# ns1labs/pktvisor

Hardware: AMD Instinct MI355X
Metric: Mpkt/s device-resident (Net+DNS handler parse) (higher is better)
Workload: dtype u8; 1 GPU; C2: Net+DNS handlers, 64 B UDP (Eth+IPv4+UDP+22 B), Zipf IPs, host_spec 10.x.x.x/8; records_per_gpu=10000000, handlers=net v1 + dns v1 (default groups), parallelism=dp1

## Files before the change

pktvisor_amd/csrc/pv_host.cpp:

```cpp
#include "pv_host.h"

namespace {

int parse_host_spec(pv_ctx *c, const char *spec)
{
    if (!spec) return 0;
    std::string s = spec;
    size_t pos = 0;
    while (pos < s.size()) {
        size_t e = s.find(',', pos);
        std::string host = s.substr(pos, e == std::string::npos ? std::string::npos : e - pos);
        pos = e == std::string::npos ? s.size() : e + 1;
        if (host.empty()) continue;
        size_t d = host.find('/');
        if (d == std::string::npos) return c->fail(PV_EINVAL, "invalid CIDR: %s", host.c_str());
        std::string ip = host.substr(0, d), cs = host.substr(d + 1);
        if (cs.empty() || !std::all_of(cs.begin(), cs.end(), ::isdigit)) return c->fail(PV_EINVAL, "invalid CIDR: %s", host.c_str());
        int cidr = atoi(cs.c_str());
        if (ip.find(':') != std::string::npos) {
            if (cidr < 0 || cidr > 128) return c->fail(PV_EINVAL, "invalid CIDR: %s", host.c_str());
            if (c->nets.n6 >= PV_MAX_SUBNETS) return c->fail(PV_EINVAL, "too many host subnets");
            uint8_t a[16];
            if (inet_pton(AF_INET6, ip.c_str(), a) != 1) return c->fail(PV_EINVAL, "invalid IPv6 address: %s", ip.c_str());
            memcpy(c->nets.v6_addr[c->nets.n6], a, 16);
// ... 2568 lines not shown
    if (status[ST_FLAGS] & PVF_NAMES_PENDING) {
        for (uint32_t t = 0; t < PV_TABLES; t++)
            hipLaunchKernelGGL(pv_topn_name_fix, dim3((uint32_t)c->cus * 4), dim3(256), 0, st, (const PvParams *)c->d_params, t);
        if (!hip_ok(e = hipGetLastError()) || !hip_ok(e = hipStreamSynchronize(st))) return c->hipfail(e, "pending names");
        if (getenv("PV_NAMEFIX_TRACE")) fprintf(stderr, "pv: pending top-N names written (pv_topn_name_fix)\n");
    }
    HP(4);
    {
        float ms = 0;
        if (timed && hipEventElapsedTime(&ms, c->ev_start, c->ev_stop) == hipSuccess) { c->kernel_ms += ms; c->kernel_launches++; }
    }
    if (!c->tcp_pre) {
        if (int rc = tcp_stage(c, d_recs, d_offs, n, status[ST_TSEG], status[ST_TSEG_BYTES], first_sec, false, st)) return rc;
    }
    const uint32_t gt = tcp_pass(c, P, a, a + nord, st, c->h_params + 1);
    if (gt) {
        if (P.want_events)
            hipLaunchKernelGGL(pv_xact_compact, dim3(gt), dim3(256), 0, st, (const PvParams *)c->d_params, grid,
                               status[ST_NKEYS]);
        if (!hip_ok(e = hipGetLastError())) return c->hipfail(e, "launch pv_dns_tcp");
        if (!hip_ok(e = hipMemcpyAsync(c->h_status, c->d_status, ST_RB_WORDS * 4, hipMemcpyDeviceToHost, st)) ||
            !hip_ok(e = hipStreamSynchronize(st)))
            return c->hipfail(e, "TCP DNS pass");
        memcpy(status, c->h_status, sizeof status);
    }
    for (uint32_t k = 0; k <= P.n_shift; k++) c->net.clean[P.slot_of[k]] = false;
    if (status[ST_NDNS] || gt)
        for (uint32_t k = 0; k <= P.n_dshift; k++) c->dns.clean[P.dslot_of[k]] = false;
    bool drained = false;
    if (int rc = drain_overflow(c, st, true, &drained)) return rc;
    uint32_t flags = status[ST_FLAGS];
    if (drained && !hip_ok(e = hipMemcpy(&flags, c->d_status + ST_FLAGS, 4, hipMemcpyDeviceToHost))) return c->hipfail(e, "status");
    if (flags & PVF_TABLE_FULL) return c->fail(PV_ECAPACITY, "top-N table full: raise table_log2");
    if (flags & PVF_ARENA_FULL) return c->fail(PV_ECAPACITY, "top-N name arena full");
    if (getenv("PV_TSTAMPS")) {
        std::vector<uint64_t> tv(65536 + (2u << c->reg_log2) * 8);
        if (hip_ok(hipMemcpy(tv.data(), c->d_stamps + (1u << 20), tv.size() * 8, hipMemcpyDeviceToHost))) {
            double cs[8] = {0}, ms[8] = {0};
            uint64_t nm = 0;
            const uint32_t cg = P.cb_grid;
            for (uint32_t w = 0; w < cg; w++)
                for (int k = 0; k < 8; k++) cs[k] += (double)tv[w * 8 + k];
            for (uint32_t w = 0; w < (2u << c->reg_log2); w++) {
                const uint64_t *m = &tv[65536 + w * 8];
                if (!m[0] && !m[1]) continue;
                nm++;
                for (int k = 0; k < 8; k++) ms[k] += (double)m[k];
            }
            fprintf(stderr, "pv_tstamps combine (%u wg): init=%.0f insert=%.0f count=%.0f scan=%.0f out=%.0f | merge (%lu wg): "
                            "runs=%.0f load=%.0f insert=%.0f names=%.0f wb=%.0f\n",
                    cg, cs[0] / cg, cs[1] / cg, cs[2] / cg, cs[3] / cg, cs[4] / cg, (unsigned long)nm,
                    ms[0] / std::max<uint64_t>(nm, 1), ms[1] / std::max<uint64_t>(nm, 1), ms[2] / std::max<uint64_t>(nm, 1),
                    ms[3] / std::max<uint64_t>(nm, 1), ms[4] / std::max<uint64_t>(nm, 1));
            hipMemset(c->d_stamps + (1u << 20), 0, tv.size() * 8);
        }
        std::vector<uint64_t> nv((size_t)reg_grid * 4);
        int khz = 0;
        hipDeviceGetAttribute(&khz, hipDeviceAttributeWallClockRate, c->device);
        if (lean && hip_ok(hipMemcpy(nv.data(), c->d_stamps + (1u << 20) + (1u << 18), nv.size() * 8, hipMemcpyDeviceToHost)) && nv[0]) {
            uint64_t first = ~0ull;
            std::vector<uint32_t> xcc(reg_grid);
            for (uint32_t w = 0; w < reg_grid; w++) {
                xcc[w] = (uint32_t)(nv[w * 4] >> 60);
                nv[w * 4] &= ~(0xfull << 60);
                first = std::min(first, nv[w * 4]);
            }
            const double us = khz > 0 ? 1000.0 / khz : 0.01;
            fprintf(stderr, "pv_tstamps net (%u wg, %s):", reg_grid, fuse ? "fused" : "pair");
            static const char *nm[4] = {"start", "net_end", "handover", "end"};
            for (int k = 0; k < (fuse ? 4 : 2); k++) {
                std::vector<double> v;
                for (uint32_t w = 0; w < reg_grid; w++)
                    if (nv[w * 4 + k]) v.push_back((double)(nv[w * 4 + k] - first) * us);
                if (v.empty()) continue;
                std::sort(v.begin(), v.end());
                fprintf(stderr, " %s min=%.2f med=%.2f max=%.2f us", nm[k], v.front(), v[v.size() / 2], v.back());
            }
            fprintf(stderr, "\n");
            fprintf(stderr, "pv_tstamps net_end by xcc:");
            for (uint32_t x = 0; x < 16; x++) {
                std::vector<double> v;
                for (uint32_t w = 0; w < reg_grid; w++)
                    if (xcc[w] == x && nv[w * 4 + 1]) v.push_back((double)(nv[w * 4 + 1] - first) * us);
                if (v.empty()) continue;
                std::sort(v.begin(), v.end());
                fprintf(stderr, " x%u(n=%zu) %.0f/%.0f/%.0f", x, v.size(), v.front(), v[v.size() / 2], v.back());
            }
            fprintf(stderr, "\n");
            hipMemset(c->d_stamps + (1u << 20) + (1u << 18), 0, nv.size() * 8);
        }
    }
    if (getenv("PV_STAMPS")) {
        std::vector<uint64_t> stv((size_t)grid * 4 * 8);
        if (hip_ok(hipMemcpy(stv.data(), c->d_stamps, stv.size() * 8, hipMemcpyDeviceToHost))) {
            double sum[8] = {0};
            for (size_t w = 0; w < (size_t)grid * 4; w++)
                for (int k = 0; k < 8; k++) sum[k] += (double)stv[w * 8 + k];
            fprintf(stderr, "pv_stamps (mean cycles per wave, %u wave tiles/wg):", P.wt_per_block);
            static const char *nm[8] = {"slot", "commit", "barA", "issue", "parse", "lane", "barB", "flush"};
            for (int k = 0; k < 8; k++) fprintf(stderr, " %s=%.0f", nm[k], sum[k] / (grid * 4.0));
            fprintf(stderr, "\n");
        }
    }
    HP(5);
    if (int rc = pair_stage(c, P, status[ST_NEV], status[ST_NKEYS], status[ST_NRESP], n, st,
                            (uint64_t)(grid + gt) * P.wt_per_block * 64u))
        return rc;
// ... 1757 lines not shown
```

pktvisor_amd/csrc/pv_kernels.hip:

```cpp
#include <cstring>
#include <hip/hip_runtime.h>
#include <rocprim/rocprim.hpp>
#include <stdint.h>

#include "pv_layout.h"
#include "pv_geodb.h"

#define PV_BLOCK 256
#define PV_C __attribute__((address_space(4)))
#ifdef PV_STAMPS
#define STAMP_DECL                                                                           \
    uint64_t st_acc[8] = {0, 0, 0, 0, 0, 0, 0, 0};                                          \
    uint64_t st_prev = __builtin_amdgcn_s_memtime();
#define STAMP(k)                                                                             \
    {                                                                                        \
        const uint64_t now = __builtin_amdgcn_s_memtime();                                   \
        st_acc[k] += now - st_prev;                                                          \
        st_prev = now;                                                                       \
    }
#define STAMP_FLUSH                                                                          \
    if ((threadIdx.x & 63) == 0)                                                             \
        for (int k_ = 0; k_ < 8; k_++) P.stamps[((uint64_t)blockIdx.x * (blockDim.x / 64) + threadIdx.x / 64) * 8 + k_] = st_acc[k_];
#else
#define STAMP_DECL
// ... 1719 lines not shown
    Parsed o;
    o.caplen = f.caplen;
    o.sec = r.w[0];
    o.nsec = ts_nano ? (int32_t)r.w[1] : (int32_t)(r.w[1] * 1000u);
    o.frame = off + 16;
    o.l3 = 4; o.l4 = (uint8_t)f.l4; o.has4 = 1; o.has6 = 0; o.syn = (uint8_t)f.syn; o.dir = (uint8_t)f.dir;
    o.v4 = o.frame + 14; o.v6 = 0;
    o.l4off = f.l4 ? o.frame + 34 : 0;
    o.l4len = f.l4 ? f.l4len : 0;
    return o;
}
__device__ __forceinline__ SlowOut net_slow_p(const PvParams *__restrict__ Pp, const SAcc R, uint64_t off, uint64_t i)
{
    PV_CREF(PvParams) P = *(const PV_C PvParams *)Pp;
    NetK K;
    K.recs = P.recs; K.offs = P.offs; K.n = P.n; K.rec_bytes = P.rec_bytes; K.gbase = P.gbase;
    K.sum = P.sum; K.cpc = P.cpc; K.iplog = P.iplog; K.dq = P.dq; K.flags = P.flags;
    K.n_shift = 0; K.skip_before = 0; K.slot0 = P.slot_of[0];
    K.net_groups = P.net_groups; K.dbg = 0; K.net_filter_all = 0;
    K.n_dshift = P.n_dshift; K.dskip_before = P.dskip_before;
    K.tcp_emit = P.tcp_emit; K.tseg_cap = P.tseg_cap; K.tseg = P.tseg; K.tseg_cnt = P.tseg_cnt; K.tmask = P.tmask;
    K.ndeep_net = nullptr; K.ndeep_dns = nullptr; K.gfilt = nullptr;
    return net_slow_body(R, parse_cfg(P), P, K, off, i, K.slot0, true);
}

#ifndef PV_REG_MINW
#define PV_REG_MINW 2
#endif
struct NetRegState {
    uint32_t hist[PV_HBINS];
    uint32_t nd, nx, ns;
    int64_t dord[PV_MAX_SHIFTS];
};
__device__ __forceinline__ void win_load(const PV_G uint8_t *recs, uint32_t off, uint4 (&W)[5])
{
    const PV_G uint4 *p = reinterpret_cast<const PV_G uint4 *>(recs + (off & ~3u));
#pragma unroll
    for (int j = 0; j < 5; j++) W[j] = p[j];
}
__device__ __forceinline__ void win_words(const uint4 (&W)[5], uint32_t sh, RecW &r)
{
    uint32_t x[17];
#pragma unroll
    for (int k = 0; k < 4; k++) { x[4 * k] = W[k].x; x[4 * k + 1] = W[k].y; x[4 * k + 2] = W[k].z; x[4 * k + 3] = W[k].w; }
    x[16] = W[4].x;
#pragma unroll
    for (int j = 0; j < 16; j++) r.w[j] = __builtin_amdgcn_alignbyte(x[j + 1], x[j], sh);
}
#ifdef PV_TSTAMPS
#define PV_TST_NET ((1u << 20) + (1u << 18))
#define TST_WALL(P, k) if (threadIdx.x == 0) (P).stamps[PV_TST_NET + 4ull * blockIdx.x + (k)] = wall_clock64();
#define TST_WALL_XCC(P) \
    if (threadIdx.x == 0) (P).stamps[PV_TST_NET + 4ull * blockIdx.x] = (wall_clock64() & ~(0xfull << 60)) | (uint64_t)__builtin_amdgcn_s_getreg(20 | (3 << 11)) << 60;
#else
#define TST_WALL_XCC(P)
#define TST_WALL(P, k)
#endif
__device__ __forceinline__ void net_ranges(PV_CREF(PvParams) P, bool contig, uint32_t &lb0, uint32_t &lb1, uint32_t &step)
{
    lb0 = blockIdx.x; lb1 = P.grid_main; step = gridDim.x;
    if (contig) { lb0 = min(blockIdx.x * P.cb_fan, P.grid_main); lb1 = min(lb0 + P.cb_fan, P.grid_main); step = 1; }
}
#define PV_RING_CTRS 12
struct FuseRing {
    struct Sec {
        uint32_t ip[PV_RING_SLOTS][PV_WT];
        uint64_t dm[PV_RING_SLOTS];
    } sec[2];
    uint32_t ctr[PV_RING_CTRS];
    uint32_t bad;
    uint32_t pad;
};
#ifdef PV_RING_SYNC_TAIL
#define PV_RING_LDS_TAIL false
#else
#define PV_RING_LDS_TAIL true
#endif
template <bool LDS>
__device__ __forceinline__ void tail_barrier()
{
    if constexpr (LDS) lds_barrier();
    else __syncthreads();
}
template <uint32_t NW, bool TC = false, bool FUSE = false, bool RING = false>
__device__ __forceinline__ void net_fast_reg(const PvParams *__restrict__ Pp, FuseRing *ring = nullptr)
{
    static_assert(!RING || (FUSE && TC && NW == PV_RING_WAVES), "the ring is the fused kernel's");
    PV_CREF(PvParams) P = *(const PV_C PvParams *)Pp;
    __shared__ NetRegState S;
    TST_WALL_XCC(P)
    const uint32_t wave = __builtin_amdgcn_readfirstlane(threadIdx.x >> 6), lane = threadIdx.x & 63;
    for (uint32_t b = threadIdx.x; b < PV_HBINS; b += (FUSE ? 64u * NW : blockDim.x)) S.hist[b] = 0;
    if (threadIdx.x == 0) { S.nd = 0; S.nx = 0; S.ns = 0; }
    if (threadIdx.x < PV_MAX_SHIFTS) S.dord[threadIdx.x] = P.dpos[threadIdx.x];
    if constexpr (RING) {
        if (threadIdx.x < PV_RING_CTRS) ring->ctr[threadIdx.x] = 0;
        if (threadIdx.x == 0) ring->bad = 0;
    }
    __syncthreads();
    const PV_G uint8_t *const recs = P.recs;
    const bool compact = P.ip_compact;
    const PV_G uint32_t *const offs = P.offs;
    const uint64_t n = P.n, last = n - 1;
    const uint32_t slot = P.slot_of[0];
    const uint32_t groups = P.net_groups;
    const bool tops = groups & PV_NET_TOP_IPS_BIT, card = groups & PV_NET_CARDINALITY_BIT;
    const uint32_t ts_nano = P.ts_nano;
    HostNets h;
    {
// ... 806 lines not shown
{
    for (uint64_t j0 = threadIdx.x; j0 < n; j0 += (uint64_t)U * blockDim.x) {
        decltype(ld(0)) v[U];
#pragma unroll
        for (int u = 0; u < U; u++) {
            const uint64_t j = j0 + (uint64_t)u * blockDim.x;
            if (j < n) v[u] = ld(j);
        }
#pragma unroll
        for (int u = 0; u < U; u++) {
            const uint64_t j = j0 + (uint64_t)u * blockDim.x;
            if (j < n) body(j, v[u]);
        }
    }
}
#define PV_E16(q) reinterpret_cast<const PV_G ulonglong2 *>(q)
#define PV_W_IP4 (1u << 31)

__device__ __forceinline__ uint32_t ip4_coupon(uint32_t ip)
{
    uint64_t h1, h2;
    murmur_8((uint64_t)(int64_t)(int32_t)ip, h1, h2);
    return cpc_coupon(h1, h2);
}

__device__ __forceinline__ uint32_t entry_table(uint64_t e0)
{
    return PV_TSLOT((uint32_t)(e0 >> 60), PV_KEY_METRIC(e0 & ((1ull << 60) - 1)));
}
__device__ __forceinline__ uint32_t log_region(PV_CREF(PvParams) P, uint64_t e0)
{
    return tregion(P, tkey_hash(e0 & ((1ull << 60) - 1)));
}
__device__ __forceinline__ uint64_t pv_run_word(uint32_t start, uint32_t cnt, uint32_t tabs)
{
    return (uint64_t)start | (uint64_t)cnt << 24 | (uint64_t)((tabs | tabs >> PV_SLOTS) & 0xffffu) << 48;
}
__device__ __forceinline__ uint32_t run_key(PV_CREF(PvParams) P, uint64_t e0)
{
    return (entry_table(e0) / PV_SLOTS) << P.reg_log2 | log_region(P, e0);
}
__device__ __forceinline__ uint64_t ip_tkey(uint64_t e)
{
    return PV_KEY_METRIC(e & ((1ull << 60) - 1)) == TM_IPV4 ? (e & (0xffull << 56)) | (e & 0xffffffffull) : e;
}

#define PV_W_CNT ((1u << 29) - 1)
#ifndef PV_CB_U
#define PV_CB_U 8
#endif
#ifndef PV_CB_OSWEEP
#define PV_CB_OSWEEP 4
#endif
#ifndef PV_MG_U
#define PV_MG_U 8
#endif
template <uint32_t CN, uint32_t NR>
struct CombState {
    union {
        struct {
            alignas(16) uint64_t key[CN];
            uint32_t cnt[CN];
            uint32_t rep[CN];
        };
        struct {
            alignas(16) uint32_t ckey[2 * CN];
            uint32_t ccnt[CN];
            uint32_t crep[CN];
        };
    };
    uint32_t h[NR];
    uint32_t tb[NR / 2];
    uint32_t wsum[PV_CB_THREADS / 64];
    uint32_t nsp;
    uint32_t hm;
};
__device__ __forceinline__ ulonglong2 comb_entry(uint64_t ck, uint32_t w, uint32_t rep)
{
    uint64_t e0 = ck;
    if (PV_KEY_METRIC(ck & ((1ull << 60) - 1)) == TM_IPV4 && !PV_IS_V2_IP4(ck & ((1ull << 60) - 1))) {
        e0 = ip_tkey(ck);
        w = PV_W_IP4 | ((uint32_t)(ck >> 32) & 1u) << 30 | ((uint32_t)(ck >> 33) & 1u) << 29 | (w & PV_W_CNT);
    }
    return make_ulonglong2(e0, (uint64_t)w | ((uint64_t)rep << 32));
}
template <class St>
__device__ __forceinline__ uint32_t comb_count(PV_CREF(PvParams) P, St &S, uint64_t e0)
{
    const uint32_t r = run_key(P, e0);
    atomicAdd(&S.h[r], 1u);
    const uint32_t bit = 1u << ((entry_table(e0) & 15u) + 16u * (r & 1u));
    if (!(S.tb[r >> 1] & bit)) atomicOr(&S.tb[r >> 1], bit);
    return r;
}
#ifndef PV_CB_BUCKET
#define PV_CB_BUCKET 1
#endif
template <class St>
__device__ __forceinline__ bool comb_bucket(PV_CREF(PvParams) P, St &S, uint32_t b, uint64_t ck, uint32_t w, uint32_t rep)
{
    const uint4 *kp = reinterpret_cast<const uint4 *>(&S.key[b]);
    const uint4 lo = kp[0], hi = kp[1];
    const uint64_t cur4[4] = {(uint64_t)lo.x | ((uint64_t)lo.y << 32), (uint64_t)lo.z | ((uint64_t)lo.w << 32),
                              (uint64_t)hi.x | ((uint64_t)hi.y << 32), (uint64_t)hi.z | ((uint64_t)hi.w << 32)};
#pragma unroll
    for (int j = 0; j < 4; j++) {
// ... 129 lines not shown
            return true;
        }
    }
    return false;
}
template <uint32_t CN2, class St>
__device__ __forceinline__ void comb_cadd_pre(PV_CREF(PvParams) P, St &S, PV_G ulonglong2 *sp, uint32_t ip, uint32_t dir,
                                              uint32_t base, uint32_t rel, uint32_t pos, uint32_t cur0, uint32_t rel0)
{
    uint32_t cur = cur0;
    if (cur == 0) {
        const uint32_t prev = atomicCAS(&S.ckey[pos], 0u, ip);
        cur = prev == 0 ? ip : prev;
        rel0 = 0xffffffffu;
    }
    if (cur == ip) {
        comb_chit(S, pos, rel, rel0);
        return;
    }
    for (uint32_t g = 1; g <= 4; g++)
        if (comb_cbucket(S, ((pos & ~7u) + 8u * g) & (CN2 - 1), pos & 1u, ip, rel)) return;
    comb_spill(P, S, sp, P.ip_base | (uint64_t)dir << 32 | ip, 1u, base + rel);
}

template <bool LDS = false>
__device__ __forceinline__ uint32_t block_excl_scan(uint32_t v, uint32_t *wsum, uint32_t &total)
{
    const uint32_t lane = threadIdx.x & 63, wv = threadIdx.x >> 6, nw = (blockDim.x + 63) >> 6;
    uint32_t incl = v;
#pragma unroll
    for (int o = 1; o < 64; o <<= 1) {
        const uint32_t t = __shfl_up(incl, o, 64);
        if (lane >= (uint32_t)o) incl += t;
    }
    if (lane == 63) wsum[wv] = incl;
    tail_barrier<LDS>();
    uint32_t base = 0, tot = 0;
    for (uint32_t k = 0; k < nw; k++) {
        const uint32_t s = wsum[k];
        if (k < wv) base += s;
        tot += s;
    }
    tail_barrier<LDS>();
    total = tot;
    return base + incl - v;
}

template <bool FUSE, class T>
__device__ __forceinline__ T ld_own(const PV_G T *p)
{
    if constexpr (FUSE) return __hip_atomic_load(p, __ATOMIC_RELAXED, __HIP_MEMORY_SCOPE_AGENT);
    else return *p;
}
template <bool RING>
__device__ __forceinline__ FuseRing *fuse_ring()
{
    if constexpr (RING) {
        __shared__ FuseRing r;
        return &r;
    } else
        return nullptr;
}
template <uint32_t CN, class St>
__device__ __forceinline__ void comb_init(St &S, uint32_t nreg, uint32_t tid, uint32_t nt)
{
    for (uint32_t j = tid; j < CN; j += nt) { S.key[j] = 0; S.cnt[j] = 0; S.rep[j] = 0xffffffffu; }
    for (uint32_t r = tid; r < nreg; r += nt) {
        S.h[r] = 0;
        if (!(r & 1)) S.tb[r >> 1] = 0;
    }
    if (tid == 0) S.nsp = 0;
}
template <uint32_t CN, class St>
__device__ __forceinline__ void comb_crange_own(PV_CREF(PvParams) P, St &S, PV_G ulonglong2 *sp, uint32_t gr, uint32_t cbase,
                                                uint32_t tid, uint32_t bd)
{
    const PV_G uint32_t *ip4 = P.iplog32;
    uint64_t a, z;
    wg_records(P, gr, a, z);
    const uint32_t nn = (uint32_t)(z - a), ra = (uint32_t)(a - cbase);
    for (uint32_t j0 = tid; j0 < nn; j0 += PV_CB_U * bd) {
        uint32_t ipv[PV_CB_U];
        uint64_t dw[PV_CB_U];
#pragma unroll
        for (int u = 0; u < PV_CB_U; u++) {
            const uint32_t j = j0 + u * bd;
            ipv[u] = j < nn ? ld_own<true>(ip4 + a + j) : 0u;
            dw[u] = j < nn ? ld_own<true>(P.ipdir + ((a + j) >> 6)) : 0ull;
        }
        uint32_t dir[PV_CB_U], pos[PV_CB_U], cur[PV_CB_U], rp[PV_CB_U];
#pragma unroll
        for (int u = 0; u < PV_CB_U; u++) {
            const uint64_t r = a + j0 + (uint64_t)u * bd;
            dir[u] = (uint32_t)(dw[u] >> (r & 63)) & 1u;
            pos[u] = comb_cpos<2 * CN>(ipv[u], dir[u]);
            cur[u] = ipv[u] ? S.ckey[pos[u]] : 0u;
            rp[u] = ipv[u] ? (S.crep[pos[u] >> 1] >> (16u * (pos[u] & 1u))) & 0xffffu : 0u;
        }
#pragma unroll
        for (int u = 0; u < PV_CB_U; u++)
            if (ipv[u]) comb_cadd_pre<2 * CN>(P, S, sp, ipv[u], dir[u], cbase, ra + j0 + u * bd, pos[u], cur[u], rp[u]);
    }
}
template <uint32_t CN, uint32_t NR, bool FUSE = false, bool RING = false>
__device__ __forceinline__ void topn_combine(PV_CREF(PvParams) P, const PvParams *__restrict__ Pp = nullptr)
{
    using St = CombState<CN, NR>;
    __shared__ St S;
    constexpr uint32_t CK = 16;
    constexpr bool CAN = CN * 2 == CK * PV_CB_THREADS && NR <= 2048;
    bool early = false;
    if constexpr (FUSE) {
        static_assert(sizeof(St) + sizeof(NetRegState) <= 160 * 1024, "pv_net_combine_plain: the Net state and the combine table in one CU's LDS");
        constexpr uint32_t NETW = 4;
        const uint32_t e0 = blockIdx.x * P.cb_fan, e1 = min(e0 + P.cb_fan, P.grid_main);
        uint64_t ea = 0, ez = 0, eb, ey = 0;
        if (e1 > e0) { wg_records(P, e0, ea, ez); wg_records(P, e1 - 1, eb, ey); }
#ifndef PV_FUSE_NO_EARLY
        early = CAN && P.cb_compact && e1 > e0 + 1 && P.ip_compact && (P.net_groups & PV_NET_TOP_IPS_BIT) && blockDim.x == PV_CB_THREADS &&
                ey - ea <= 65535;
#endif
        FuseRing *const ring = fuse_ring<RING>();
        if constexpr (RING) {
            static_assert(CAN && sizeof(St) + sizeof(NetRegState) + sizeof(FuseRing) <= 160 * 1024, "pv_net_combine_ring: the ring beside them");
            static_assert(PV_CB_THREADS == 64 * (NETW + PV_RING_SLOTS), "an inserting thread a slot's lane");
            early = true;
        }
        if (__builtin_amdgcn_readfirstlane(threadIdx.x >> 6) < NETW) {
            net_fast_reg<NETW, true, true, RING>(Pp, ring);
            if constexpr (!(RING && PV_RING_LDS_TAIL)) __builtin_amdgcn_s_waitcnt(PV_WAIT_VMCNT0);
        } else if constexpr (RING) {
            const uint32_t tid = threadIdx.x - 64u * NETW, nt = blockDim.x - 64u * NETW;
            const uint32_t slot = tid >> 6, lane = tid & 63;
            PV_G ulonglong2 *const sp = reinterpret_cast<PV_G ulonglong2 *>(P.tp_buf) + (uint64_t)e0 * P.mq_cap;
            const uint64_t nwt = (P.n + PV_WT - 1) / PV_WT;
            lds_barrier();
            comb_init<CN>(S, 2u << P.reg_log2, tid, nt);
            uint32_t secn = 0;
            for (uint32_t gr = e0; gr < e1; gr++) {
                const uint64_t wbeg = (uint64_t)gr * P.wt_per_block, wend = min<uint64_t>(wbeg + P.wt_per_block, nwt);
                const uint32_t ns = pv_ring_sections(wend > wbeg ? (uint32_t)(wend - wbeg) : 0u);
                const uint32_t ra = (uint32_t)(wbeg * PV_WT - ea);
                for (uint32_t s = 0; s < ns; s++, secn++) {
                    lds_barrier();
                    const FuseRing::Sec &rs = ring->sec[secn & 1];
                    const uint32_t ip = rs.ip[slot][lane];
                    if (ip) {
                        const uint32_t dir = (uint32_t)(rs.dm[slot] >> lane) & 1u, pos = comb_cpos<2 * CN>(ip, dir);
                        comb_cadd_pre<2 * CN>(P, S, sp, ip, dir, (uint32_t)ea, ra + (pv_ring_tile(s, slot) * PV_WT + lane), pos, S.ckey[pos],
                                              (S.crep[pos >> 1] >> (16u * (pos & 1u))) & 0xffffu);
                    }
                }
                lds_barrier();
                lds_barrier();
            }
            __builtin_amdgcn_s_waitcnt(PV_WAIT_VMCNT0);
            lds_barrier();
        } else {
            const uint32_t tid = threadIdx.x - 64u * NETW, nt = blockDim.x - 64u * NETW;
            lds_barrier();
            comb_init<CN>(S, 2u << P.reg_log2, tid, nt);
            for (uint32_t gr = e0; gr < e1; gr++) {
                lds_barrier();
                lds_barrier();
                if (early && gr + 1 < e1)
                    comb_crange_own<CN>(P, S, reinterpret_cast<PV_G ulonglong2 *>(P.tp_buf) + (uint64_t)e0 * P.mq_cap, gr, (uint32_t)ea, tid, nt);
            }
            lds_barrier();
        }
        tail_barrier<RING && PV_RING_LDS_TAIL>();
        TST_WALL(P, 2)
    }
    constexpr bool LT = RING && PV_RING_LDS_TAIL;
    if constexpr (!FUSE) {
        if (P.plain_chain && (*P.n_dns | *P.n_slow)) return;
    }
    TST_DECL
// ... 64 lines not shown
                }
            }
        }
    } else
    for (uint32_t gr = g0; gr < g1; gr++) {
    const uint32_t cnt = ld_own<FUSE>(P.mq_cnt + gr);
    const PV_G uint64_t *q = P.mq + (uint64_t)gr * P.mq_cap * 2;
    batched<8>(cnt, [&](uint64_t j) { return PV_E16(q)[j]; },
               [&](uint64_t, ulonglong2 e) { comb_add<CN>(P, S, sp, e.x, (uint32_t)e.y, (uint32_t)(e.y >> 32)); });
    if (P.net_groups & PV_NET_TOP_IPS_BIT) {
        uint64_t a, z;
        wg_records(P, gr, a, z);
        const PV_G uint64_t *ipl = P.iplog + a;
        if (P.ip_compact) {
            const PV_G uint32_t *ip4 = P.iplog32;
            const uint64_t nn = z - a, bd = blockDim.x;
            const uint64_t ipb = P.ip_base;
            for (uint64_t j0 = threadIdx.x; j0 < nn; j0 += (uint64_t)PV_CB_U * bd) {
                uint32_t ipv[PV_CB_U];
                uint64_t dw[PV_CB_U];
#pragma unroll
                for (int u = 0; u < PV_CB_U; u++) {
                    const uint64_t j = j0 + (uint64_t)u * bd;
                    ipv[u] = j < nn ? ld_own<FUSE>(ip4 + a + j) : 0u;
                    dw[u] = j < nn ? ld_own<FUSE>(P.ipdir + ((a + j) >> 6)) : 0ull;
                }
                uint64_t ck[PV_CB_U], cur[PV_CB_U];
                uint32_t pos[PV_CB_U], rp[PV_CB_U];
#pragma unroll
                for (int u = 0; u < PV_CB_U; u++) {
                    const uint64_t r = a + j0 + (uint64_t)u * bd;
                    ck[u] = ipb | ((dw[u] >> (r & 63)) & 1) << 32 | ipv[u];
                    pos[u] = (uint32_t)(fmix64(ck[u]) >> 20) & (CN - 1);
                    cur[u] = ipv[u] ? S.key[pos[u]] : 0ull;
                    rp[u] = ipv[u] ? S.rep[pos[u]] : 0u;
                }
#pragma unroll
                for (int u = 0; u < PV_CB_U; u++)
                    if (ipv[u]) comb_add_pre<CN>(P, S, sp, ck[u], 1u, (uint32_t)(a + j0 + (uint64_t)u * bd), pos[u], cur[u], rp[u]);
            }
            const uint32_t nx = ld_own<FUSE>(P.ipx_cnt + gr);
            for (uint32_t q = threadIdx.x; q < nx; q += blockDim.x)
                comb_add<CN>(P, S, sp, ld_own<FUSE>(ipl + q), 1u, ld_own<FUSE>(P.ipx_rep + a + q));
        } else {
            batched<PV_CB_U>(z - a, [&](uint64_t j) { return ipl[j]; }, [&](uint64_t j, uint64_t e) {
                if (e) comb_add<CN>(P, S, sp, e, 1u, (uint32_t)(a + j));
            });
        }
    }
    }
    if (threadIdx.x == 0) S.hm = 0;
    tail_barrier<LT>();
    TST(1)
    uint32_t rk[CK / 2] = {};
    if (compact) {
        if constexpr (CAN) {
            const uint64_t tk = P.ip_base & (0xffull << 56);
#pragma unroll
            for (uint32_t k = 0; k < CK; k++) {
                const uint32_t ip = S.ckey[threadIdx.x + k * PV_CB_THREADS];
                const uint32_t r = ip ? comb_count(P, S, tk | ip) : 0u;
                rk[k / 2] = k & 1 ? rk[k / 2] | r << 16 : r;
            }
        }
    } else
    for (uint32_t j = threadIdx.x; j < CN; j += blockDim.x)
        if (S.key[j]) comb_count(P, S, comb_entry(S.key[j], S.cnt[j], S.rep[j]).x);
    tail_barrier<LT>();
    TST(2)
    const uint32_t per = (nreg + blockDim.x - 1) / blockDim.x;
    const uint32_t r0 = min(threadIdx.x * per, nreg), r1 = min(r0 + per, nreg);
    uint32_t s = 0;
    for (uint32_t r = r0; r < r1; r++) s += S.h[r];
    {
        const uint32_t hb = s ? 1u << (r0 >> P.reg_log2) : 0u;
        const uint64_t b0 = __ballot(hb & 1), b1 = __ballot(hb & 2);
        if ((threadIdx.x & 63) == 0 && (b0 | b1)) atomicOr(&S.hm, (b0 ? 1u : 0u) | (b1 ? 2u : 0u));
    }
    uint32_t total;
    uint32_t run = block_excl_scan<LT>(s, S.wsum, total);
    const uint32_t hm = S.hm;
    if (threadIdx.x < 2 && ((hm >> threadIdx.x) & 1)) atomicOr(P.tp_hands, 1u << threadIdx.x);
    if (threadIdx.x == 0) P.cb_hm[blockIdx.x] = hm;
    const uint32_t ng8 = (P.cb_grid + 7) / 8;
    PV_G uint64_t *col = P.cb_run + (blockIdx.x % 8) * ng8 + blockIdx.x / 8;
    for (uint32_t r = r0; r < r1; r++) {
        const uint32_t c = S.h[r];
        if ((hm >> (r >> P.reg_log2)) & 1) col[(uint64_t)r * 8 * ng8] = pv_run_word(run, c, (S.tb[r >> 1] >> (16u * (r & 1u))) & 0xffffu);
        S.h[r] = run;
        run += c;
    }
    lds_barrier();
    TST(3)
    if (compact) {
        if constexpr (CAN) {
#pragma unroll 1
            for (uint32_t q = 0; q < PV_CB_OSWEEP; q++)
#pragma unroll
            for (uint32_t k = 0; k < CK; k++) {
                const uint32_t j = threadIdx.x + k * PV_CB_THREADS, sh = 16u * (j & 1u);
                const uint32_t ip = S.ckey[j];
                if (!ip) continue;
                if (PV_CB_OSWEEP > 1 && ((((rk[k / 2] >> (16u * (k & 1u))) & 0xffffu) * PV_CB_OSWEEP) >> P.reg_log2) != q) continue;
                const uint64_t ck = P.ip_base | (uint64_t)((j ^ (uint32_t)__popc(ip)) & 1u) << 32 | ip;
                const ulonglong2 e = comb_entry(ck, (S.ccnt[j >> 1] >> sh) & 0xffffu, cbase + ((S.crep[j >> 1] >> sh) & 0xffffu));
                out[atomicAdd(&S.h[(rk[k / 2] >> (16u * (k & 1u))) & 0xffffu], 1u)] = e;
            }
        }
    } else
    for (uint32_t j = threadIdx.x; j < CN; j += blockDim.x)
        if (S.key[j]) {
            const ulonglong2 e = comb_entry(S.key[j], S.cnt[j], S.rep[j]);
            out[atomicAdd(&S.h[run_key(P, e.x)], 1u)] = e;
        }
    const uint32_t nsp = S.nsp;
    batched<8>(nsp, [&](uint64_t j) { return sp[j]; },
               [&](uint64_t, ulonglong2 e) { out[atomicAdd(&S.h[run_key(P, e.x)], 1u)] = e; });
    if (threadIdx.x == 0) P.cb_cnt[blockIdx.x] = total;
#ifdef PV_TSTAMPS
    __syncthreads();
#endif
    TST(4)
    TST_FLUSH(0)
    if constexpr (FUSE) { TST_WALL(P, 3) }
}
#ifndef PV_CB_CN
#define PV_CB_CN 8192
#endif
static_assert(PV_SLOTS == 16, "pv_topn_combine folds a table bit to 16 bits a region");
extern "C" __global__ void __launch_bounds__(PV_CB_THREADS) pv_topn_combine(const PvParams *__restrict__ Pp)
{
    PV_CREF(PvParams) P = *(const PV_C PvParams *)Pp;
    topn_combine<PV_CB_CN, 2048>(P);
}
extern "C" __global__ void __launch_bounds__(PV_CB_THREADS) pv_net_combine_plain(const PvParams *__restrict__ Pp)
{
    PV_CREF(PvParams) P = *(const PV_C PvParams *)Pp;
    topn_combine<PV_CB_CN, 2048, true>(P, Pp);
}
extern "C" __global__ void __launch_bounds__(PV_CB_THREADS) pv_net_combine_ring(const PvParams *__restrict__ Pp)
{
    PV_CREF(PvParams) P = *(const PV_C PvParams *)Pp;
    topn_combine<PV_CB_CN, 2048, true, true>(P, Pp);
}
extern "C" __global__ void __launch_bounds__(256) pv_net_iplog(const PvParams *__restrict__ Pp)
{
// ... 15 lines not shown
        win_words(W, off & 3, rw);
        const FastRec f = fast_fields(rw, h);
        const uint32_t ip = f.dir == 0 ? rw.at(42) : rw.at(46);
        const bool ipok = i < n && f.ok != 0 && f.dir != 2 && ip != 0;
        const uint64_t dbit = __ballot(ipok && f.dir == 1);
        P.iplog32[i] = ipok ? ip : 0u;
        if (lane == 0) P.ipdir[t] = dbit;
    }
}
extern "C" __global__ void __launch_bounds__(PV_CB_THREADS) pv_topn_combine_r12(const PvParams *__restrict__ Pp)
{
    PV_CREF(PvParams) P = *(const PV_C PvParams *)Pp;
    topn_combine<2048, 2u << PV_MAX_REGIONS_LOG2>(P);
}

#define PV_MG_THREADS 512
#ifndef PV_MG_U2
#define PV_MG_U2 4
#endif
#ifndef PV_MG_SEEN
#define PV_MG_SEEN 1
#endif
#define PV_MG_NN 640
#define PV_CREATED (1ull << 63)
#define PV_MV4 (1ull << 62)
#define PV_MN1 (0xffffffull << 32)
#define PV_DL0 (0xffffffffull << 32)
__device__ __forceinline__ bool mv4_key(uint64_t k) { return PV_KEY_METRIC(k) == TM_IPV4 && !((k >> 40) & 1); }
__device__ __forceinline__ uint64_t mv4_norm(uint64_t w) { return w & ~(PV_CREATED | ((w & PV_MV4) ? PV_MN1 : 0ull)); }
struct MergeState {
    alignas(16) uint64_t key[PV_RS];
    uint64_t dl[PV_RS];
    uint32_t nrep[PV_MG_NN];
    uint16_t nidx[PV_MG_NN];
    uint32_t nnew, nbase, ncr;
    uint32_t ip4c;
};
struct MergeRuns {
    uint32_t start[PV_MAX_GRID + 8];
    uint32_t pref[PV_MAX_GRID + 9];
    uint16_t list[PV_MAX_GRID + 8];
    uint32_t wsum[16];
    uint32_t tabs;
};
static_assert(2 * PV_MG_THREADS >= (PV_MAX_GRID + 7) / 8 * 8, "two runs per merge thread");
static_assert(sizeof(MergeState) + sizeof(MergeRuns) <= 80 * 1024, "pv_topn_merge: two workgroups per CU");
extern "C" uint32_t pv_topn_merge_threads() { return PV_MG_THREADS; }
extern "C" __global__ void __launch_bounds__(PV_MG_THREADS) __attribute__((amdgpu_waves_per_eu(4))) pv_topn_merge(const PvParams *__restrict__ Pp)
{
    PV_CREF(PvParams) P = *(const PV_C PvParams *)Pp;
    const uint32_t rk = blockIdx.x;
    const uint32_t r = rk & ((1u << P.reg_log2) - 1);
    const uint32_t hd = rk >> P.reg_log2;
    if (P.plain_chain && (*P.n_dns | *P.n_slow)) return;
    if (!((*P.tp_hands >> hd) & 1)) return;
    if (P.xmerge && (r < P.x_lo || r >= P.x_hi)) return;
    __shared__ MergeRuns U;
    __shared__ MergeState S;
    TST_DECL
    const uint32_t ng8 = (P.cb_grid + 7) / 8, ng = 8 * ng8;
    const uint64_t lcap = (uint64_t)P.cb_fan * P.mq_cap;
    const uint32_t rsl = P.tcap_log2 - P.reg_log2;
    const uint32_t rs = 1u << rsl;
    const uint32_t tbg = hd ? PV_SLOTS + P.dslot_of[0] : P.slot_of[0];
    const uint64_t rbg = ((uint64_t)tbg << P.tcap_log2) + ((uint64_t)r << rsl);
    const bool pf = rs == PV_RS;
    if (pf) {
        static_assert(PV_RS * 8 == 32 * 1024 && PV_MG_THREADS == 512, "four pieces per wave");
        const uint32_t wv = threadIdx.x >> 6, ln = threadIdx.x & 63;
#pragma unroll
        for (int q = 0; q < 4; q++) {
            const uint32_t pc = wv * 4 + q;
            dma16(P.tkeys + rbg + pc * 128 + ln * 2, lds_addr(&S.key[pc * 128]));
        }
    }
    uint32_t n;
    {
        uint32_t c0 = 0, c1 = 0, tb = 0;
        if (threadIdx.x == 0) U.tabs = 0;
        const uint32_t i0 = 2 * threadIdx.x;
        if (i0 < ng) {
            const ulonglong2 v = *reinterpret_cast<const PV_G ulonglong2 *>(P.cb_run + (uint64_t)rk * ng + i0);
            const uint32_t w0 = (i0 % ng8) * 8 + i0 / ng8, w1 = ((i0 + 1) % ng8) * 8 + (i0 + 1) / ng8;
            const bool h0 = w0 < P.cb_grid && ((P.cb_hm[w0] >> hd) & 1);
            const bool h1 = w1 < P.cb_grid && ((P.cb_hm[w1] >> hd) & 1);
            U.start[i0] = (uint32_t)v.x & 0xffffffu;
            U.start[i0 + 1] = (uint32_t)v.y & 0xffffffu;
            U.list[i0] = (uint16_t)w0;
            U.list[i0 + 1] = (uint16_t)w1;
            c0 = h0 ? (uint32_t)(v.x >> 24) & 0xffffffu : 0u;
            c1 = h1 ? (uint32_t)(v.y >> 24) & 0xffffffu : 0u;
            tb = (h0 ? (uint32_t)(v.x >> 48) : 0u) | (h1 ? (uint32_t)(v.y >> 48) : 0u);
        }
        uint32_t total;
        PV_VMCNT(0);
        const uint32_t pre = block_excl_scan(c0 + c1, U.wsum, total);
        if (i0 < ng) { U.pref[i0] = pre; U.pref[i0 + 1] = pre + c0; }
        if (threadIdx.x == 0) U.pref[ng] = total;
        if (tb) atomicOr(&U.tabs, tb);
        __syncthreads();
        n = total;
    }
    TST(0)
    if (n == 0) return;
    uint32_t top = 1;
    while (top * 2 < ng) top *= 2;
    const PV_G ulonglong2 *cb = reinterpret_cast<const PV_G ulonglong2 *>(P.cb);
    auto ld = [&](uint64_t j) -> ulonglong2 {
        uint32_t lo = 0;
        for (uint32_t st = top; st; st >>= 1) {
            const uint32_t m = lo + st;
            if (m < ng && U.pref[m] <= (uint32_t)j) lo = m;
        }
        return cb[(uint64_t)U.list[lo] * lcap + U.start[lo] + ((uint32_t)j - U.pref[lo])];
    };
    static_assert(PV_TABLES <= 32, "table mask");
    constexpr uint32_t PF = PV_RS / PV_MG_THREADS;
    const bool narrow = P.n <= (1ull << 24) && !P.xmerge;
    const bool xm = P.xmerge != 0;
    const bool trust = PV_MG_SEEN && narrow && P.seen_trust;
    uint32_t tabs = U.tabs << (hd * PV_SLOTS);
    const bool one = !(tabs & (tabs - 1));
    bool fresh = true;
    while (tabs) {
        const uint32_t tb = __builtin_ctz(tabs);
        const uint32_t s = tb % PV_SLOTS;
        tabs &= tabs - 1;
        const uint64_t rbase = ((uint64_t)tb << P.tcap_log2) + ((uint64_t)r << rsl);
        if (!(pf && tb == tbg && fresh)) batched<4>(rs, [&](uint64_t i) { return P.tkeys[rbase + i]; }, [&](uint64_t i, uint64_t k) { S.key[i] = k; });
        for (uint32_t i = threadIdx.x; i < rs; i += blockDim.x) {
            const uint64_t k = S.key[i];
            if (narrow && mv4_key(k)) S.key[i] = k | PV_MV4 | PV_MN1;
            S.dl[i] = PV_DL0;
        }
        if (threadIdx.x == 0) { S.nnew = 0; S.ncr = 0; S.ip4c = 0; }
        lds_barrier();
        TST(1)
        auto ins = [&](ulonglong2 e) __attribute__((always_inline)) {
            const uint64_t e0 = e.x;
            if (!one && entry_table(e0) != tb) return;
            const uint32_t w32 = (uint32_t)e.y, rep = (uint32_t)(e.y >> 32);
            const uint64_t w = xm ? e.y : (w32 & PV_W_IP4) ? (uint64_t)(w32 & PV_W_CNT) : (uint64_t)w32;
            const uint64_t key = e0 & ((1ull << 60) - 1);
            const bool v4 = narrow && mv4_key(key);
            const bool card = !xm && (w32 & PV_W_IP4) && ((w32 >> 29) & 1);
            if (card && !v4) S.ip4c = 1;
            const uint64_t pk = v4 ? key | PV_MV4 : key;
            uint32_t pos = (uint32_t)tkey_hash(key) & (rs - 1);
            for (int probe = 0; probe < PV_PROBES; probe++) {
                uint64_t cur = S.key[pos];
                bool created = false;
                if (cur == 0) {
                    const uint64_t nw = pk | (v4 ? PV_MN1 : 0ull) | PV_CREATED;
                    const uint64_t prev = atomicCAS((unsigned long long *)&S.key[pos], 0ull, (unsigned long long)nw);
                    created = prev == 0;
                    cur = created ? nw : prev;
                }
// ... 79 lines not shown
                    if (xm && PV_KEY_METRIC(kk[q] & ~PV_CREATED) != TM_IPV4) P.taux[rbase + i] = 0;
                }
                uint64_t nf = 0;
                if ((kk[q] & PV_MV4) && dd[q]) {
                    const uint32_t m0 = (uint32_t)(S.dl[i] >> 32), m1 = (uint32_t)(kk[q] >> 32) & 0xffffffu;
                    const uint64_t seen = trust ? cc[q] : 0;
                    const bool s0 = m0 != 0xffffffffu && !(seen & PV_CNT_SEEN_SRC);
                    const bool s1 = m1 != 0xffffffu && !(seen & PV_CNT_SEEN_DST);
                    if (s0 || s1) {
                        const uint32_t cp = ip4_coupon((uint32_t)kk[q]);
                        if (s0) cpc_min(P, s, CPC_SRC, cp, (int64_t)(P.gbase + m0));
                        if (s1) cpc_min(P, s, CPC_DST, cp, (int64_t)(P.gbase + m1));
                        if (trust) nf = (s0 ? PV_CNT_SEEN_SRC : 0ull) | (s1 ? PV_CNT_SEEN_DST : 0ull);
                    }
                }
                if (dd[q]) st_nt<PV_NT_MERGE, uint64_t>(P.tcnt + rbase + i, (cc[q] + dd[q]) | nf);
            }
        }
        if (threadIdx.x == 0 && S.ncr) atomicAdd(&P.tab_live[tb], S.ncr);
        if (S.ip4c) {
            lds_barrier();
            for (uint32_t i = threadIdx.x; i < rs; i += blockDim.x) S.dl[i] = ~0ull;
            lds_barrier();
            batched<PV_MG_U2>(n, ld, [&](uint64_t, ulonglong2 e) {
                const uint32_t w32 = (uint32_t)e.y, rep = (uint32_t)(e.y >> 32), d = (w32 >> 30) & 1;
                if (!(w32 & PV_W_IP4) || !((w32 >> 29) & 1) || (!one && entry_table(e.x) != tb)) return;
                const uint64_t key = e.x & ((1ull << 60) - 1);
                uint32_t pos = (uint32_t)tkey_hash(key) & (rs - 1);
                for (int probe = 0; probe < PV_PROBES; probe++) {
                    const uint64_t cur = S.key[pos] & ~PV_CREATED;
                    if (cur == key) {
                        atomicMin(reinterpret_cast<uint32_t *>(&S.dl[pos]) + d, rep);
                        return;
                    }
                    if (cur == 0) break;
                    pos = (pos + 1) & (rs - 1);
                }
                cpc_min(P, s, d ? CPC_DST : CPC_SRC, ip4_coupon((uint32_t)key), (int64_t)(P.gbase + rep));
            });
            lds_barrier();
            for (uint32_t i = threadIdx.x; i < rs; i += blockDim.x) {
                const uint64_t m = S.dl[i];
                if (m == ~0ull) continue;
                const uint32_t cp = ip4_coupon((uint32_t)S.key[i]);
                if ((uint32_t)m != 0xffffffffu) cpc_min(P, s, CPC_SRC, cp, (int64_t)(P.gbase + (uint32_t)m));
                if ((uint32_t)(m >> 32) != 0xffffffffu) cpc_min(P, s, CPC_DST, cp, (int64_t)(P.gbase + (uint32_t)(m >> 32)));
            }
        }
        if (tabs) lds_barrier();
        TST(4)
        fresh = false;
    }
    TST_FLUSH(65536)
}

__device__ __forceinline__ uint32_t x_owner(uint32_t r, uint32_t reg_log2, uint32_t W) { return (uint32_t)(((uint64_t)r * W) >> reg_log2); }
__device__ __forceinline__ uint32_t x_lo(uint32_t d, uint32_t reg_log2, uint32_t W) { return (uint32_t)((((uint64_t)d << reg_log2) + W - 1) / W); }
#define PV_XC(hd, r, slot, reg_log2) ((((uint32_t)(hd) << (reg_log2)) + (r)) * PV_SLOTS + (slot))

extern "C" __global__ void __launch_bounds__(256) pv_topn_xcount(const PvParams *__restrict__ Pp, PvXTabs T, uint32_t *__restrict__ cnt)
{
    PV_CREF(PvParams) P = *(const PV_C PvParams *)Pp;
    __shared__ uint32_t wsum[16];
    const uint32_t r = blockIdx.x & ((1u << P.reg_log2) - 1), tb = T.tb[blockIdx.x >> P.reg_log2];
    const uint32_t rs = 1u << (P.tcap_log2 - P.reg_log2);
    uint32_t c = 0;
    if (x_owner(r, P.reg_log2, T.W) != T.me) {
        const PV_G uint64_t *k = P.tkeys + ((uint64_t)tb << P.tcap_log2) + ((uint64_t)r << (P.tcap_log2 - P.reg_log2));
        for (uint32_t i = threadIdx.x; i < rs; i += blockDim.x) c += k[i] != 0;
    }
    uint32_t tot;
    block_excl_scan(c, wsum, tot);
    if (threadIdx.x == 0) cnt[PV_XC(tb / PV_SLOTS, r, tb % PV_SLOTS, P.reg_log2)] = tot;
}

extern "C" __global__ void __launch_bounds__(1024) pv_topn_xscan(uint32_t reg_log2, uint32_t W, const uint32_t *__restrict__ cnt,
                                                                 uint32_t *__restrict__ off, uint32_t *__restrict__ hdr)
{
    __shared__ uint32_t wsum[16];
    const uint32_t E = (2u << reg_log2) * PV_SLOTS, per = (E + blockDim.x - 1) / blockDim.x;
    const uint32_t p0 = min(threadIdx.x * per, E), p1 = min(p0 + per, E);
    auto cell = [&](uint32_t p) {
        const uint32_t d = x_owner(p / (2 * PV_SLOTS), reg_log2, W);
        const uint32_t lo = x_lo(d, reg_log2, W), len = x_lo(d + 1, reg_log2, W) - lo;
        const uint32_t rem = p - 2 * PV_SLOTS * lo, hd = rem / (PV_SLOTS * len);
        return PV_XC(hd, lo + (rem % (PV_SLOTS * len)) / PV_SLOTS, rem % PV_SLOTS, reg_log2);
    };
    uint32_t s = 0;
    for (uint32_t p = p0; p < p1; p++) s += cnt[cell(p)];
    uint32_t tot;
    uint32_t at = block_excl_scan(s, wsum, tot);
    for (uint32_t p = p0; p < p1; p++) {
        const uint32_t i = cell(p), c = cnt[i];
        off[i] = at;
        hdr[p] = c;
        at += c;
    }
}

extern "C" __global__ void __launch_bounds__(256) pv_topn_xwrite(const PvParams *__restrict__ Pp, PvXTabs T, const uint32_t *__restrict__ off,
                                                                 ulonglong2 *__restrict__ out)
{
    PV_CREF(PvParams) P = *(const PV_C PvParams *)Pp;
    __shared__ uint32_t wsum[16];
    const uint32_t r = blockIdx.x & ((1u << P.reg_log2) - 1), tb = T.tb[blockIdx.x >> P.reg_log2];
    if (x_owner(r, P.reg_log2, T.W) == T.me) return;
// ... 1596 lines not shown
```

Before: 33910 Mpkt/s.

## Write ring combine output in slot order via LDS inverse index window

In the ring-fused combine kernel, each compacted key now gets its output position through an LDS atomic on the per-slot histogram. An inverse index maps positions back to keys in LDS windows of 5120 entries, so the output entries are written to global memory in contiguous, coalesced order. This replaces the previous compact output loop when PV_RING_OUT_SWEEPS is 0, the default. The RingOut union overlays the inverse buffer on the FuseRing LDS storage. The change also adds wall-clock timestamp instrumentation to the merge kernel, which compiles only under PV_TSTAMPS.

```diff
diff --git a/pktvisor_amd/csrc/pv_host.cpp b/pktvisor_amd/csrc/pv_host.cpp
--- a/pktvisor_amd/csrc/pv_host.cpp
+++ b/pktvisor_amd/csrc/pv_host.cpp
@@ -2644,7 +2644,34 @@
                     cg, cs[0] / cg, cs[1] / cg, cs[2] / cg, cs[3] / cg, cs[4] / cg, (unsigned long)nm,
                     ms[0] / std::max<uint64_t>(nm, 1), ms[1] / std::max<uint64_t>(nm, 1), ms[2] / std::max<uint64_t>(nm, 1),
                     ms[3] / std::max<uint64_t>(nm, 1), ms[4] / std::max<uint64_t>(nm, 1));
+            fprintf(stderr, "pv_tstamps merge head: guards=%.0f wait=%.0f scan=%.0f\n", ms[5] / std::max<uint64_t>(nm, 1),
+                    ms[6] / std::max<uint64_t>(nm, 1), ms[0] / std::max<uint64_t>(nm, 1));
             hipMemset(c->d_stamps + (1u << 20), 0, tv.size() * 8);
+        }
+        std::vector<uint64_t> mv((size_t)(2u << c->reg_log2) * 2);
+        int mkhz = 0;
+        hipDeviceGetAttribute(&mkhz, hipDeviceAttributeWallClockRate, c->device);
+        if (hip_ok(hipMemcpy(mv.data(), c->d_stamps + (1u << 20) + (1u << 19), mv.size() * 8, hipMemcpyDeviceToHost))) {
+            const double us = mkhz > 0 ? 1000.0 / mkhz : 0.01;
+            const uint32_t hw = 1u << c->reg_log2;
+            uint64_t first = ~0ull;
+            for (uint32_t w = 0; w < 2 * hw; w++)
+                if (mv[2 * w]) first = std::min(first, mv[2 * w]);
+            for (uint32_t h = 0; h < 2 && first != ~0ull; h++) {
+                uint64_t s0 = ~0ull, s1 = 0, e1 = 0;
+                uint32_t k = 0;
+                for (uint32_t w = h * hw; w < (h + 1) * hw; w++) {
+                    if (!mv[2 * w]) continue;
+                    k++;
+                    s0 = std::min(s0, mv[2 * w]);
+                    s1 = std::max(s1, mv[2 * w]);
+                    e1 = std::max(e1, mv[2 * w + 1]);
+                }
+                if (k)
+                    fprintf(stderr, "pv_tstamps merge wall %s half (%u wg): first start=%.2f last start=%.2f last end=%.2f us\n",
+                            h ? "DNS" : "Net", k, (double)(s0 - first) * us, (double)(s1 - first) * us, (double)(e1 - first) * us);
+            }
+            hipMemset(c->d_stamps + (1u << 20) + (1u << 19), 0, mv.size() * 8);
         }
         std::vector<uint64_t> nv((size_t)reg_grid * 4);
         int khz = 0;
diff --git a/pktvisor_amd/csrc/pv_kernels.hip b/pktvisor_amd/csrc/pv_kernels.hip
--- a/pktvisor_amd/csrc/pv_kernels.hip
+++ b/pktvisor_amd/csrc/pv_kernels.hip
@@ -1795,9 +1795,12 @@
 #define TST_WALL(P, k) if (threadIdx.x == 0) (P).stamps[PV_TST_NET + 4ull * blockIdx.x + (k)] = wall_clock64();
 #define TST_WALL_XCC(P) \
     if (threadIdx.x == 0) (P).stamps[PV_TST_NET + 4ull * blockIdx.x] = (wall_clock64() & ~(0xfull << 60)) | (uint64_t)__builtin_amdgcn_s_getreg(20 | (3 << 11)) << 60;
+#define PV_TST_MG ((1u << 20) + (1u << 19))
+#define TST_MG_WALL(P, k) if (threadIdx.x == 0) (P).stamps[PV_TST_MG + 2ull * blockIdx.x + (k)] = wall_clock64();
 #else
 #define TST_WALL_XCC(P)
 #define TST_WALL(P, k)
+#define TST_MG_WALL(P, k)
 #endif
 __device__ __forceinline__ void net_ranges(PV_CREF(PvParams) P, bool contig, uint32_t &lb0, uint32_t &lb1, uint32_t &step)
 {
@@ -2710,6 +2713,9 @@
 #ifndef PV_CB_OSWEEP
 #define PV_CB_OSWEEP 4
 #endif
+#ifndef PV_RING_OUT_SWEEPS
+#define PV_RING_OUT_SWEEPS 0
+#endif
 #ifndef PV_MG_U
 #define PV_MG_U 8
 #endif
@@ -2945,14 +2951,27 @@
     if constexpr (FUSE) return __hip_atomic_load(p, __ATOMIC_RELAXED, __HIP_MEMORY_SCOPE_AGENT);
     else return *p;
 }
+#define PV_RING_OUT_W 5120
+#define PV_RING_OUT_NONE 0xffffu
+union RingOut {
+    FuseRing r;
+    uint16_t inv[PV_RING_OUT_W];
+};
+static_assert(PV_RING_OUT_W % PV_CB_THREADS == 0, "pv_net_combine_ring: whole turns of the workgroup a window");
 template <bool RING>
-__device__ __forceinline__ FuseRing *fuse_ring()
+__device__ __forceinline__ RingOut *ring_out()
 {
     if constexpr (RING) {
-        __shared__ FuseRing r;
+        __shared__ RingOut r;
         return &r;
     } else
         return nullptr;
+}
+template <bool RING>
+__device__ __forceinline__ FuseRing *fuse_ring()
+{
+    if constexpr (RING) return &ring_out<RING>()->r;
+    else return nullptr;
 }
 template <uint32_t CN, class St>
 __device__ __forceinline__ void comb_init(St &S, uint32_t nreg, uint32_t tid, uint32_t nt)
@@ -3015,7 +3034,8 @@
 #endif
         FuseRing *const ring = fuse_ring<RING>();
         if constexpr (RING) {
-            static_assert(CAN && sizeof(St) + sizeof(NetRegState) + sizeof(FuseRing) <= 160 * 1024, "pv_net_combine_ring: the ring beside them");
+            static_assert(CAN && sizeof(St) + sizeof(NetRegState) + sizeof(RingOut) <= 160 * 1024, "pv_net_combine_ring: the ring beside them");
+            static_assert(2 * CN <= PV_RING_OUT_NONE, "a table slot and the sentinel in 16 bits");
             static_assert(PV_CB_THREADS == 64 * (NETW + PV_RING_SLOTS), "an inserting thread a slot's lane");
             early = true;
         }
@@ -3186,6 +3206,9 @@
     if (threadIdx.x == 0) S.hm = 0;
     tail_barrier<LT>();
     TST(1)
+    constexpr bool WOUT = RING && !PV_RING_OUT_SWEEPS;
+    if constexpr (WOUT)
+        for (uint32_t p = threadIdx.x; p < PV_RING_OUT_W; p += PV_CB_THREADS) ring_out<RING>()->inv[p] = PV_RING_OUT_NONE;
     uint32_t rk[CK / 2] = {};
     if (compact) {
         if constexpr (CAN) {
@@ -3193,7 +3216,7 @@
 #pragma unroll
             for (uint32_t k = 0; k < CK; k++) {
                 const uint32_t ip = S.ckey[threadIdx.x + k * PV_CB_THREADS];
-                const uint32_t r = ip ? comb_count(P, S, tk | ip) : 0u;
+                const uint32_t r = ip ? comb_count(P, S, tk | ip) : WOUT ? 0xffffu : 0u;
                 rk[k / 2] = k & 1 ? rk[k / 2] | r << 16 : r;
             }
         }
@@ -3226,6 +3249,47 @@
     }
     lds_barrier();
     TST(3)
+    if constexpr (WOUT) {
+#pragma unroll
+        for (uint32_t k = 0; k < CK; k++) {
+            const uint32_t r = (rk[k / 2] >> (16u * (k & 1u))) & 0xffffu;
+            const uint32_t p = r != 0xffffu ? atomicAdd(&S.h[r], 1u) : PV_RING_OUT_NONE;
+            rk[k / 2] = k & 1 ? (rk[k / 2] & 0xffffu) | p << 16 : (rk[k / 2] & 0xffff0000u) | p;
+        }
+        uint16_t *const inv = ring_out<RING>()->inv;
+#pragma unroll 1
+        for (uint32_t base = 0; base < total; base += PV_RING_OUT_W) {
+#pragma unroll
+            for (uint32_t k = 0; k < CK; k++) {
+                const uint32_t p = (rk[k / 2] >> (16u * (k & 1u))) & 0xffffu;
+                if (p != PV_RING_OUT_NONE && p - base < PV_RING_OUT_W) inv[p - base] = (uint16_t)(threadIdx.x + k * PV_CB_THREADS);
+            }
+            lds_barrier();
+            constexpr uint32_t WT = PV_RING_OUT_W / PV_CB_THREADS;
+            uint32_t j[WT], ip[WT], cc[WT], cr[WT];
+#pragma unroll
+            for (uint32_t t = 0; t < WT; t++) {
+                const uint32_t p = threadIdx.x + t * PV_CB_THREADS;
+                j[t] = base + p < total ? inv[p] : PV_RING_OUT_NONE;
+            }
+#pragma unroll
+            for (uint32_t t = 0; t < WT; t++) {
+                const uint32_t s = j[t] != PV_RING_OUT_NONE ? j[t] : 0u;
+                inv[threadIdx.x + t * PV_CB_THREADS] = PV_RING_OUT_NONE;
+                ip[t] = S.ckey[s];
+                cc[t] = S.ccnt[s >> 1];
+                cr[t] = S.crep[s >> 1];
+            }
+#pragma unroll
+            for (uint32_t t = 0; t < WT; t++) {
+                if (j[t] == PV_RING_OUT_NONE) continue;
+                const uint32_t sh = 16u * (j[t] & 1u);
+                const uint64_t ck = P.ip_base | (uint64_t)((j[t] ^ (uint32_t)__popc(ip[t])) & 1u) << 32 | ip[t];
+                out[base + threadIdx.x + t * PV_CB_THREADS] = comb_entry(ck, (cc[t] >> sh) & 0xffffu, cbase + ((cr[t] >> sh) & 0xffffu));
+            }
+            if (base + PV_RING_OUT_W < total) lds_barrier();
+        }
+    } else
     if (compact) {
         if constexpr (CAN) {
 #pragma unroll 1
@@ -3347,12 +3411,14 @@
     const uint32_t rk = blockIdx.x;
     const uint32_t r = rk & ((1u << P.reg_log2) - 1);
     const uint32_t hd = rk >> P.reg_log2;
-    if (P.plain_chain && (*P.n_dns | *P.n_slow)) return;
-    if (!((*P.tp_hands >> hd) & 1)) return;
+    TST_MG_WALL(P, 0)
+    TST_DECL
+    if (P.plain_chain && (*P.n_dns | *P.n_slow)) { TST_MG_WALL(P, 1) return; }
+    if (!((*P.tp_hands >> hd) & 1)) { TST_MG_WALL(P, 1) return; }
     if (P.xmerge && (r < P.x_lo || r >= P.x_hi)) return;
     __shared__ MergeRuns U;
     __shared__ MergeState S;
-    TST_DECL
+    TST(5)
     const uint32_t ng8 = (P.cb_grid + 7) / 8, ng = 8 * ng8;
     const uint64_t lcap = (uint64_t)P.cb_fan * P.mq_cap;
     const uint32_t rsl = P.tcap_log2 - P.reg_log2;
@@ -3389,6 +3455,7 @@
         }
         uint32_t total;
         PV_VMCNT(0);
+        TST(6)
         const uint32_t pre = block_excl_scan(c0 + c1, U.wsum, total);
         if (i0 < ng) { U.pref[i0] = pre; U.pref[i0 + 1] = pre + c0; }
         if (threadIdx.x == 0) U.pref[ng] = total;
@@ -3397,7 +3464,7 @@
         n = total;
     }
     TST(0)
-    if (n == 0) return;
+    if (n == 0) { TST_MG_WALL(P, 1) return; }
     uint32_t top = 1;
     while (top * 2 < ng) top *= 2;
     const PV_G ulonglong2 *cb = reinterpret_cast<const PV_G ulonglong2 *>(P.cb);
@@ -3583,6 +3650,7 @@
         fresh = false;
     }
     TST_FLUSH(65536)
+    TST_MG_WALL(P, 1)
 }
 
 __device__ __forceinline__ uint32_t x_owner(uint32_t r, uint32_t reg_log2, uint32_t W) { return (uint32_t)(((uint64_t)r * W) >> reg_log2); }
```

Result: faster. 34270 Mpkt/s, median of 4 (+1.0%).
